# ZHKKKe/PixelSSL

Measured on NVIDIA H100. Metric: images/sec DeepLab-v2-R101 MT 513x513 bs16, higher is better.
Workload: dtype f16x3 (fp16 pairs, fp32 accumulate)

## Files before the change

pixelssl_b200/csrc/conv_tc.cu:

```cuda
#include "common.cuh"
#include <cuda.h>
#include <cstdlib>

typedef CUresult (*EncodeTiledFn)(CUtensorMap*, CUtensorMapDataType, cuuint32_t, void*, const cuuint64_t*,
                                  const cuuint64_t*, const cuuint32_t*, const cuuint32_t*, CUtensorMapInterleave,
                                  CUtensorMapSwizzle, CUtensorMapL2promotion, CUtensorMapFloatOOBfill);
static EncodeTiledFn get_encode() {
    static EncodeTiledFn fn = nullptr;
    if (!fn) {
        void* p = nullptr;
        cudaDriverEntryPointQueryResult q;
        if (cudaGetDriverEntryPoint("cuTensorMapEncodeTiled", &p, cudaEnableDefault, &q) == cudaSuccess &&
            q == cudaDriverEntryPointSuccess)
            fn = (EncodeTiledFn)p;
    }
    return fn;
}

static int make_act_map(CUtensorMap* m, const void* base, int C, int W, int H, int N, int bw, int bh, int estride = 1, int f16 = 0) {
    EncodeTiledFn enc = get_encode();
    if (!enc) return PXL_ERR_UNSUPPORTED;
    const cuuint64_t eb = f16 ? 2 : 4;
    cuuint64_t dims[4] = {(cuuint64_t)C, (cuuint64_t)W, (cuuint64_t)H, (cuuint64_t)N};
    cuuint64_t strides[3] = {(cuuint64_t)C * eb, (cuuint64_t)W * C * eb, (cuuint64_t)H * W * C * eb};
// ... 6 lines not shown
    return r == CUDA_SUCCESS ? 0 : PXL_ERR_BAD_ARG;
}

static int make_w_map(CUtensorMap* m, const void* base, int64_t K, int rows, int bn, int f16 = 0) {
    EncodeTiledFn enc = get_encode();
    if (!enc) return PXL_ERR_UNSUPPORTED;
    cuuint64_t dims[2] = {(cuuint64_t)K, (cuuint64_t)rows};
    cuuint64_t strides[1] = {(cuuint64_t)K * (f16 ? 2 : 4)};
    cuuint32_t box[2] = {(cuuint32_t)(f16 ? 64 : 32), (cuuint32_t)bn};
    cuuint32_t es[2] = {1, 1};
    CUresult r = enc(m, f16 ? CU_TENSOR_MAP_DATA_TYPE_FLOAT16 : CU_TENSOR_MAP_DATA_TYPE_FLOAT32, 2, (void*)base, dims, strides, box, es,
                     CU_TENSOR_MAP_INTERLEAVE_NONE, CU_TENSOR_MAP_SWIZZLE_128B, CU_TENSOR_MAP_L2_PROMOTION_L2_256B,
                     CU_TENSOR_MAP_FLOAT_OOB_FILL_NONE);
    return r == CUDA_SUCCESS ? 0 : PXL_ERR_BAD_ARG;
}

__device__ __forceinline__ uint32_t smem_u32(const void* p) { return (uint32_t)__cvta_generic_to_shared(p); }

__device__ __forceinline__ void mbar_init(uint64_t* bar, uint32_t count) {
    asm volatile("mbarrier.init.shared::cta.b64 [%0], %1;" ::"r"(smem_u32(bar)), "r"(count));
}
__device__ __forceinline__ void mbar_expect_tx(uint64_t* bar, uint32_t bytes) {
    asm volatile("mbarrier.arrive.expect_tx.shared::cta.b64 _, [%0], %1;" ::"r"(smem_u32(bar)), "r"(bytes) : "memory");
}
__device__ __forceinline__ void mbar_arrive(uint64_t* bar) {
    asm volatile("mbarrier.arrive.shared::cta.b64 _, [%0];" ::"r"(smem_u32(bar)) : "memory");
}
__device__ __forceinline__ bool mbar_try_wait(uint64_t* bar, uint32_t parity) {
    uint32_t ok;
    asm volatile(
        "{\n\t.reg .pred p;\n\t"
        "mbarrier.try_wait.parity.shared::cta.b64 p, [%1], %2;\n\t"
        "selp.u32 %0, 1, 0, p;\n\t}"
        : "=r"(ok)
        : "r"(smem_u32(bar)), "r"(parity)
        : "memory");
    return ok != 0;
}
__device__ __forceinline__ bool mbar_wait(uint64_t* bar, uint32_t parity, int* flag, int code) {
    for (uint32_t spin = 0; spin < (1u << 22); ++spin) {
        if (mbar_try_wait(bar, parity)) return true;
        if ((spin & 1023u) == 1023u && *(volatile int*)flag != 0) return false;
    }
    atomicCAS(flag, 0, code);
    return false;
}
__device__ __forceinline__ void tma_load_4d(void* dst, const CUtensorMap* map, uint64_t* bar, int c0, int c1, int c2, int c3) {
    asm volatile(
        "cp.async.bulk.tensor.4d.shared::cluster.global.mbarrier::complete_tx::bytes [%0], [%1, {%3, %4, %5, %6}], [%2];"
        ::"r"(smem_u32(dst)), "l"(map), "r"(smem_u32(bar)), "r"(c0), "r"(c1), "r"(c2), "r"(c3)
        : "memory");
}
__device__ __forceinline__ void tma_load_2d(void* dst, const CUtensorMap* map, uint64_t* bar, int c0, int c1) {
    asm volatile(
        "cp.async.bulk.tensor.2d.shared::cluster.global.mbarrier::complete_tx::bytes [%0], [%1, {%3, %4}], [%2];"
        ::"r"(smem_u32(dst)), "l"(map), "r"(smem_u32(bar)), "r"(c0), "r"(c1)
        : "memory");
}
__device__ __forceinline__ bool elect_one() {
    uint32_t pred = 0;
    asm volatile(
        "{\n\t.reg .b32 rx;\n\t.reg .pred px;\n\t"
        "elect.sync rx|px, 0xffffffff;\n\t"
        "@px mov.s32 %0, 1;\n\t}"
        : "+r"(pred));
    return pred != 0;
}
__device__ __forceinline__ void named_bar(int id, int count) {
    asm volatile("bar.sync %0, %1;" ::"r"(id), "r"(count) : "memory");
}
__device__ __forceinline__ void fence_async_smem() { asm volatile("fence.proxy.async.shared::cta;" ::: "memory"); }

__device__ __forceinline__ uint64_t sw128_desc(uint32_t smem_addr, uint32_t lbo_bytes = 16) {
    uint64_t d = 0;
    d |= (uint64_t)((smem_addr & 0x3FFFF) >> 4);
    d |= (uint64_t)((lbo_bytes >> 4) & 0x3FFF) << 16;
    d |= (uint64_t)(1024 >> 4) << 32;
    d |= (uint64_t)1 << 62;
    return d;
}
__device__ __forceinline__ void wg_arrive() { asm volatile("wgmma.fence.sync.aligned;" ::: "memory"); }
__device__ __forceinline__ void wg_commit() { asm volatile("wgmma.commit_group.sync.aligned;" ::: "memory"); }
__device__ __forceinline__ void wg_wait0() { asm volatile("wgmma.wait_group.sync.aligned 0;" ::: "memory"); }
template <int R>
__device__ __forceinline__ void fence_regs(float (&d)[R]) {
#pragma unroll
    for (int i = 0; i < R; ++i) asm volatile("" : "+f"(d[i])::"memory");
}

template <int N, int KIND>
__device__ __forceinline__ void wgmma_op(float (&d)[N / 2], uint64_t da, uint64_t db, int scale_d);
template <> __device__ __forceinline__ void wgmma_op<32, 0>(float (&d)[16], uint64_t da, uint64_t db, int scale_d) {
    asm volatile(
        "{\n\t.reg .pred p;\n\tsetp.ne.b32 p, %18, 0;\n\t"
        "wgmma.mma_async.sync.aligned.m64n32k8.f32.tf32.tf32 {%0, %1, %2, %3, %4, %5, %6, %7, %8, %9, %10, %11, %12, %13, %14, %15}, %16, %17, p, 1, 1;\n\t}"
        : "+f"(d[0]), "+f"(d[1]), "+f"(d[2]), "+f"(d[3]), "+f"(d[4]), "+f"(d[5]), "+f"(d[6]), "+f"(d[7]), "+f"(d[8]), "+f"(d[9]), "+f"(d[10]), "+f"(d[11]), "+f"(d[12]), "+f"(d[13]), "+f"(d[14]), "+f"(d[15])
        : "l"(da), "l"(db), "r"(scale_d));
}
template <> __device__ __forceinline__ void wgmma_op<64, 0>(float (&d)[32], uint64_t da, uint64_t db, int scale_d) {
    asm volatile(
        "{\n\t.reg .pred p;\n\tsetp.ne.b32 p, %34, 0;\n\t"
        "wgmma.mma_async.sync.aligned.m64n64k8.f32.tf32.tf32 {%0, %1, %2, %3, %4, %5, %6, %7, %8, %9, %10, %11, %12, %13, %14, %15, %16, %17, %18, %19, %20, %21, %22, %23, %24, %25, %26, %27, %28, %29, %30, %31}, %32, %33, p, 1, 1;\n\t}"
        : "+f"(d[0]), "+f"(d[1]), "+f"(d[2]), "+f"(d[3]), "+f"(d[4]), "+f"(d[5]), "+f"(d[6]), "+f"(d[7]), "+f"(d[8]), "+f"(d[9]), "+f"(d[10]), "+f"(d[11]), "+f"(d[12]), "+f"(d[13]), "+f"(d[14]), "+f"(d[15]), "+f"(d[16]), "+f"(d[17]), "+f"(d[18]), "+f"(d[19]), "+f"(d[20]), "+f"(d[21]), "+f"(d[22]), "+f"(d[23]), "+f"(d[24]), "+f"(d[25]), "+f"(d[26]), "+f"(d[27]), "+f"(d[28]), "+f"(d[29]), "+f"(d[30]), "+f"(d[31])
        : "l"(da), "l"(db), "r"(scale_d));
}
template <> __device__ __forceinline__ void wgmma_op<128, 0>(float (&d)[64], uint64_t da, uint64_t db, int scale_d) {
    asm volatile(
        "{\n\t.reg .pred p;\n\tsetp.ne.b32 p, %66, 0;\n\t"
        "wgmma.mma_async.sync.aligned.m64n128k8.f32.tf32.tf32 {%0, %1, %2, %3, %4, %5, %6, %7, %8, %9, %10, %11, %12, %13, %14, %15, %16, %17, %18, %19, %20, %21, %22, %23, %24, %25, %26, %27, %28, %29, %30, %31, %32, %33, %34, %35, %36, %37, %38, %39, %40, %41, %42, %43, %44, %45, %46, %47, %48, %49, %50, %51, %52, %53, %54, %55, %56, %57, %58, %59, %60, %61, %62, %63}, %64, %65, p, 1, 1;\n\t}"
        : "+f"(d[0]), "+f"(d[1]), "+f"(d[2]), "+f"(d[3]), "+f"(d[4]), "+f"(d[5]), "+f"(d[6]), "+f"(d[7]), "+f"(d[8]), "+f"(d[9]), "+f"(d[10]), "+f"(d[11]), "+f"(d[12]), "+f"(d[13]), "+f"(d[14]), "+f"(d[15]), "+f"(d[16]), "+f"(d[17]), "+f"(d[18]), "+f"(d[19]), "+f"(d[20]), "+f"(d[21]), "+f"(d[22]), "+f"(d[23]), "+f"(d[24]), "+f"(d[25]), "+f"(d[26]), "+f"(d[27]), "+f"(d[28]), "+f"(d[29]), "+f"(d[30]), "+f"(d[31]), "+f"(d[32]), "+f"(d[33]), "+f"(d[34]), "+f"(d[35]), "+f"(d[36]), "+f"(d[37]), "+f"(d[38]), "+f"(d[39]), "+f"(d[40]), "+f"(d[41]), "+f"(d[42]), "+f"(d[43]), "+f"(d[44]), "+f"(d[45]), "+f"(d[46]), "+f"(d[47]), "+f"(d[48]), "+f"(d[49]), "+f"(d[50]), "+f"(d[51]), "+f"(d[52]), "+f"(d[53]), "+f"(d[54]), "+f"(d[55]), "+f"(d[56]), "+f"(d[57]), "+f"(d[58]), "+f"(d[59]), "+f"(d[60]), "+f"(d[61]), "+f"(d[62]), "+f"(d[63])
        : "l"(da), "l"(db), "r"(scale_d));
}
template <> __device__ __forceinline__ void wgmma_op<32, 1>(float (&d)[16], uint64_t da, uint64_t db, int scale_d) {
    asm volatile(
        "{\n\t.reg .pred p;\n\tsetp.ne.b32 p, %18, 0;\n\t"
        "wgmma.mma_async.sync.aligned.m64n32k16.f32.f16.f16 {%0, %1, %2, %3, %4, %5, %6, %7, %8, %9, %10, %11, %12, %13, %14, %15}, %16, %17, p, 1, 1, 0, 0;\n\t}"
        : "+f"(d[0]), "+f"(d[1]), "+f"(d[2]), "+f"(d[3]), "+f"(d[4]), "+f"(d[5]), "+f"(d[6]), "+f"(d[7]), "+f"(d[8]), "+f"(d[9]), "+f"(d[10]), "+f"(d[11]), "+f"(d[12]), "+f"(d[13]), "+f"(d[14]), "+f"(d[15])
        : "l"(da), "l"(db), "r"(scale_d));
}
template <> __device__ __forceinline__ void wgmma_op<64, 1>(float (&d)[32], uint64_t da, uint64_t db, int scale_d) {
    asm volatile(
        "{\n\t.reg .pred p;\n\tsetp.ne.b32 p, %34, 0;\n\t"
        "wgmma.mma_async.sync.aligned.m64n64k16.f32.f16.f16 {%0, %1, %2, %3, %4, %5, %6, %7, %8, %9, %10, %11, %12, %13, %14, %15, %16, %17, %18, %19, %20, %21, %22, %23, %24, %25, %26, %27, %28, %29, %30, %31}, %32, %33, p, 1, 1, 0, 0;\n\t}"
        : "+f"(d[0]), "+f"(d[1]), "+f"(d[2]), "+f"(d[3]), "+f"(d[4]), "+f"(d[5]), "+f"(d[6]), "+f"(d[7]), "+f"(d[8]), "+f"(d[9]), "+f"(d[10]), "+f"(d[11]), "+f"(d[12]), "+f"(d[13]), "+f"(d[14]), "+f"(d[15]), "+f"(d[16]), "+f"(d[17]), "+f"(d[18]), "+f"(d[19]), "+f"(d[20]), "+f"(d[21]), "+f"(d[22]), "+f"(d[23]), "+f"(d[24]), "+f"(d[25]), "+f"(d[26]), "+f"(d[27]), "+f"(d[28]), "+f"(d[29]), "+f"(d[30]), "+f"(d[31])
        : "l"(da), "l"(db), "r"(scale_d));
}
template <> __device__ __forceinline__ void wgmma_op<128, 1>(float (&d)[64], uint64_t da, uint64_t db, int scale_d) {
    asm volatile(
        "{\n\t.reg .pred p;\n\tsetp.ne.b32 p, %66, 0;\n\t"
        "wgmma.mma_async.sync.aligned.m64n128k16.f32.f16.f16 {%0, %1, %2, %3, %4, %5, %6, %7, %8, %9, %10, %11, %12, %13, %14, %15, %16, %17, %18, %19, %20, %21, %22, %23, %24, %25, %26, %27, %28, %29, %30, %31, %32, %33, %34, %35, %36, %37, %38, %39, %40, %41, %42, %43, %44, %45, %46, %47, %48, %49, %50, %51, %52, %53, %54, %55, %56, %57, %58, %59, %60, %61, %62, %63}, %64, %65, p, 1, 1, 0, 0;\n\t}"
        : "+f"(d[0]), "+f"(d[1]), "+f"(d[2]), "+f"(d[3]), "+f"(d[4]), "+f"(d[5]), "+f"(d[6]), "+f"(d[7]), "+f"(d[8]), "+f"(d[9]), "+f"(d[10]), "+f"(d[11]), "+f"(d[12]), "+f"(d[13]), "+f"(d[14]), "+f"(d[15]), "+f"(d[16]), "+f"(d[17]), "+f"(d[18]), "+f"(d[19]), "+f"(d[20]), "+f"(d[21]), "+f"(d[22]), "+f"(d[23]), "+f"(d[24]), "+f"(d[25]), "+f"(d[26]), "+f"(d[27]), "+f"(d[28]), "+f"(d[29]), "+f"(d[30]), "+f"(d[31]), "+f"(d[32]), "+f"(d[33]), "+f"(d[34]), "+f"(d[35]), "+f"(d[36]), "+f"(d[37]), "+f"(d[38]), "+f"(d[39]), "+f"(d[40]), "+f"(d[41]), "+f"(d[42]), "+f"(d[43]), "+f"(d[44]), "+f"(d[45]), "+f"(d[46]), "+f"(d[47]), "+f"(d[48]), "+f"(d[49]), "+f"(d[50]), "+f"(d[51]), "+f"(d[52]), "+f"(d[53]), "+f"(d[54]), "+f"(d[55]), "+f"(d[56]), "+f"(d[57]), "+f"(d[58]), "+f"(d[59]), "+f"(d[60]), "+f"(d[61]), "+f"(d[62]), "+f"(d[63])
        : "l"(da), "l"(db), "r"(scale_d));
}
template <> __device__ __forceinline__ void wgmma_op<64, 2>(float (&d)[32], uint64_t da, uint64_t db, int scale_d) {
    asm volatile(
        "{\n\t.reg .pred p;\n\tsetp.ne.b32 p, %34, 0;\n\t"
        "wgmma.mma_async.sync.aligned.m64n64k16.f32.f16.f16 {%0, %1, %2, %3, %4, %5, %6, %7, %8, %9, %10, %11, %12, %13, %14, %15, %16, %17, %18, %19, %20, %21, %22, %23, %24, %25, %26, %27, %28, %29, %30, %31}, %32, %33, p, 1, 1, 1, 1;\n\t}"
        : "+f"(d[0]), "+f"(d[1]), "+f"(d[2]), "+f"(d[3]), "+f"(d[4]), "+f"(d[5]), "+f"(d[6]), "+f"(d[7]), "+f"(d[8]), "+f"(d[9]), "+f"(d[10]), "+f"(d[11]), "+f"(d[12]), "+f"(d[13]), "+f"(d[14]), "+f"(d[15]), "+f"(d[16]), "+f"(d[17]), "+f"(d[18]), "+f"(d[19]), "+f"(d[20]), "+f"(d[21]), "+f"(d[22]), "+f"(d[23]), "+f"(d[24]), "+f"(d[25]), "+f"(d[26]), "+f"(d[27]), "+f"(d[28]), "+f"(d[29]), "+f"(d[30]), "+f"(d[31])
        : "l"(da), "l"(db), "r"(scale_d));
}
template <> __device__ __forceinline__ void wgmma_op<128, 2>(float (&d)[64], uint64_t da, uint64_t db, int scale_d) {
    asm volatile(
        "{\n\t.reg .pred p;\n\tsetp.ne.b32 p, %66, 0;\n\t"
        "wgmma.mma_async.sync.aligned.m64n128k16.f32.f16.f16 {%0, %1, %2, %3, %4, %5, %6, %7, %8, %9, %10, %11, %12, %13, %14, %15, %16, %17, %18, %19, %20, %21, %22, %23, %24, %25, %26, %27, %28, %29, %30, %31, %32, %33, %34, %35, %36, %37, %38, %39, %40, %41, %42, %43, %44, %45, %46, %47, %48, %49, %50, %51, %52, %53, %54, %55, %56, %57, %58, %59, %60, %61, %62, %63}, %64, %65, p, 1, 1, 1, 1;\n\t}"
        : "+f"(d[0]), "+f"(d[1]), "+f"(d[2]), "+f"(d[3]), "+f"(d[4]), "+f"(d[5]), "+f"(d[6]), "+f"(d[7]), "+f"(d[8]), "+f"(d[9]), "+f"(d[10]), "+f"(d[11]), "+f"(d[12]), "+f"(d[13]), "+f"(d[14]), "+f"(d[15]), "+f"(d[16]), "+f"(d[17]), "+f"(d[18]), "+f"(d[19]), "+f"(d[20]), "+f"(d[21]), "+f"(d[22]), "+f"(d[23]), "+f"(d[24]), "+f"(d[25]), "+f"(d[26]), "+f"(d[27]), "+f"(d[28]), "+f"(d[29]), "+f"(d[30]), "+f"(d[31]), "+f"(d[32]), "+f"(d[33]), "+f"(d[34]), "+f"(d[35]), "+f"(d[36]), "+f"(d[37]), "+f"(d[38]), "+f"(d[39]), "+f"(d[40]), "+f"(d[41]), "+f"(d[42]), "+f"(d[43]), "+f"(d[44]), "+f"(d[45]), "+f"(d[46]), "+f"(d[47]), "+f"(d[48]), "+f"(d[49]), "+f"(d[50]), "+f"(d[51]), "+f"(d[52]), "+f"(d[53]), "+f"(d[54]), "+f"(d[55]), "+f"(d[56]), "+f"(d[57]), "+f"(d[58]), "+f"(d[59]), "+f"(d[60]), "+f"(d[61]), "+f"(d[62]), "+f"(d[63])
        : "l"(da), "l"(db), "r"(scale_d));
}

template <int BN, int F16>
__device__ __forceinline__ void mma_slice(float (&part)[BN / 2], float (&corr)[BN / 2], uint64_t da, uint64_t db, uint64_t dal,
                                          uint64_t dbl, bool split3) {
#pragma unroll
    for (int k = 0; k < 4; ++k) wgmma_op<BN, F16>(part, da + 2 * k, db + 2 * k, k);
    if (split3) {
#pragma unroll
        for (int k = 0; k < 4; ++k) wgmma_op<BN, F16>(corr, dal + 2 * k, db + 2 * k, k);
#pragma unroll
        for (int k = 0; k < 4; ++k) wgmma_op<BN, F16>(corr, da + 2 * k, dbl + 2 * k, 1);
    }
}

__device__ __forceinline__ float4 tf32_split4(float4 v, float4& lo) {
    float4 h;
    const float* vp = &v.x; float* hp = &h.x; float* lp = &lo.x;
#pragma unroll
    for (int e = 0; e < 4; ++e) {
        uint32_t u;
        asm("cvt.rna.tf32.f32 %0, %1;" : "=r"(u) : "f"(vp[e]));
        u &= 0xFFFFE000u;
        hp[e] = __uint_as_float(u);
        lp[e] = vp[e] - hp[e];
    }
    return h;
}

struct TcParams {
    int Cin, Cout, ldo, ntaps, kchunks;
    int N, OH, OW;
    int BW, BH, tilesW, tilesH;
    int stages, nsplit;
    int a_inkernel;
    int in_mul;
    int out_mul, out_offy, out_offx, outH, outW;
    int ntilesN, pix_tiles, total_tiles;
    int kc;
    float out_scale;
    int out_acc;
    short dy[PXL_MAX_TAPS], dx[PXL_MAX_TAPS], widx[PXL_MAX_TAPS];
};

#define TC_A_BYTES (128 * 128)
#define TC_MAX_STAGES 8
#define TC_THREADS 384

__device__ __forceinline__ void tc_tile_coords(const TcParams& p, int tile, int bn, int& n0, int& w0, int& h0, int& n) {
    const int nt = tile / p.pix_tiles, pix = tile - nt * p.pix_tiles;
    const int tw = pix % p.tilesW, th = (pix / p.tilesW) % p.tilesH;
    n = pix / (p.tilesW * p.tilesH);
    w0 = tw * p.BW; h0 = th * p.BH; n0 = nt * bn;
}

template <int BN, int F16>
__global__ void __launch_bounds__(TC_THREADS, 1)
conv_wg_kernel(const __grid_constant__ CUtensorMap mapA, const __grid_constant__ CUtensorMap mapAlo,
               const __grid_constant__ CUtensorMap mapB, const __grid_constant__ CUtensorMap mapBlo,
               const TcParams p, const float* __restrict__ bias, float* __restrict__ out,
               double* __restrict__ stats, int* __restrict__ err_flag, const float* __restrict__ oscale_ptr) {
    extern __shared__ __align__(1024) uint8_t smem_raw[];
    __shared__ uint64_t full_bar[TC_MAX_STAGES], empty_bar[TC_MAX_STAGES];
    __shared__ float st_warp[2][8][BN];

    uint8_t* smem = (uint8_t*)(((uintptr_t)smem_raw + 1023) & ~(uintptr_t)1023);
    constexpr int B_BYTES = BN * 128;
    constexpr int PER_OP = TC_A_BYTES + B_BYTES;
    const int stage_bytes = PER_OP * (p.nsplit == 3 ? 2 : 1);
    const int iters = p.ntaps * p.kchunks;

    if (threadIdx.x == 0) {
        for (int s = 0; s < p.stages; ++s) { mbar_init(&full_bar[s], 1); mbar_init(&empty_bar[s], 256); }
        asm volatile("fence.mbarrier_init.release.cluster;" ::: "memory");
    }
    __syncthreads();
    PXL_PDL_SYNC();

    if (threadIdx.x < 128) {
        asm volatile("setmaxnreg.dec.sync.aligned.u32 40;" ::: "memory");
        if (threadIdx.x >= 32) return;
        uint32_t tx = (uint32_t)((p.BW * p.BH * 128 + B_BYTES) * (p.nsplit == 3 ? 2 : 1));
        if (p.a_inkernel) tx -= (uint32_t)(p.BW * p.BH * 128);
        uint32_t s = 0, ph = 0;
        bool ok = true;
        for (int tile = blockIdx.x; tile < p.total_tiles && ok; tile += gridDim.x) {
            int n0, w0, h0, n;
            tc_tile_coords(p, tile, BN, n0, w0, h0, n);
            int tap = 0, c0 = 0;
            for (int it = 0; it < iters; ++it) {
                ok = __all_sync(0xffffffffu, mbar_wait(&empty_bar[s], ph ^ 1u, err_flag, 1));
                if (!ok) break;
                uint8_t* sa = smem + (size_t)s * stage_bytes;
                const int ax = w0 * p.in_mul + p.dx[tap], ay = h0 * p.in_mul + p.dy[tap];
                const int bk = p.widx[tap] * p.Cin + c0;
                if (elect_one()) {
                    mbar_expect_tx(&full_bar[s], tx);
                    tma_load_4d(sa, &mapA, &full_bar[s], c0, ax, ay, n);
                    tma_load_2d(sa + TC_A_BYTES, &mapB, &full_bar[s], bk, n0);
                    if (p.nsplit == 3) {
                        if (!p.a_inkernel) tma_load_4d(sa + PER_OP, &mapAlo, &full_bar[s], c0, ax, ay, n);
                        tma_load_2d(sa + PER_OP + TC_A_BYTES, &mapBlo, &full_bar[s], bk, n0);
                    }
                }
                __syncwarp();
                c0 += p.kc; if (c0 >= p.Cin) { c0 = 0; ++tap; }
                if (++s == (uint32_t)p.stages) { s = 0; ph ^= 1u; }
            }
        }
        return;
    }

    asm volatile("setmaxnreg.inc.sync.aligned.u32 232;" ::: "memory");
    const int ct = threadIdx.x - 128;
    const int cw = ct >> 7, t = ct & 127;
    const int warp = t >> 5, lane = t & 31;
    const float osc = p.out_scale * (oscale_ptr ? __ldg(oscale_ptr) : 1.f);
    const uint32_t smem_base = smem_u32(smem);
    const bool split3 = p.nsplit == 3;
    float acc[BN / 2], part[BN / 2], corr[BN / 2];
    uint32_t s = 0, ph = 0;
    int st_n0 = -1;
    float st_s = 0.f, st_q = 0.f;
    bool ok = true;
    auto flush_stats = [&]() {
        if (st_n0 >= 0 && ct < BN && st_n0 + ct < p.Cout && (st_s != 0.f || st_q != 0.f)) {
            atomicAdd(stats + st_n0 + ct, (double)st_s);
            atomicAdd(stats + p.Cout + st_n0 + ct, (double)st_q);
        }
        st_s = 0.f; st_q = 0.f;
    };
    for (int tile = blockIdx.x; tile < p.total_tiles && ok; tile += gridDim.x) {
        int n0, w0, h0, n;
        tc_tile_coords(p, tile, BN, n0, w0, h0, n);
        if (stats && n0 != st_n0) { flush_stats(); st_n0 = n0; }
#pragma unroll
        for (int i = 0; i < BN / 2; ++i) acc[i] = 0.f;
        for (int it = 0; it < iters; ++it) {
            ok = __all_sync(0xffffffffu, mbar_wait(&full_bar[s], ph, err_flag, 2));
            if (!ok) break;
            uint8_t* sa = smem + (size_t)s * stage_bytes;
            if (p.a_inkernel) {
                float4* a_hi = reinterpret_cast<float4*>(sa + cw * (TC_A_BYTES / 2));
                float4* a_lo = reinterpret_cast<float4*>(sa + PER_OP + cw * (TC_A_BYTES / 2));
#pragma unroll
                for (int c = 0; c < TC_A_BYTES / 2 / 16 / 128; ++c) {
                    float4 lo;
                    const float4 hi = tf32_split4(a_hi[t + c * 128], lo);
                    a_hi[t + c * 128] = hi;
                    a_lo[t + c * 128] = lo;
                }
                fence_async_smem();
                named_bar(2 + cw, 128);
            }
            const uint32_t sa32 = smem_base + s * (uint32_t)stage_bytes;
            const uint32_t arow = (uint32_t)cw * (TC_A_BYTES / 2);
            const uint64_t da = sw128_desc(sa32 + arow), db = sw128_desc(sa32 + TC_A_BYTES);
            const uint64_t dal = sw128_desc(sa32 + PER_OP + arow), dbl = sw128_desc(sa32 + PER_OP + TC_A_BYTES);
            wg_arrive();
            fence_regs(part);
            fence_regs(corr);
#pragma unroll
            for (int k = 0; k < 2; ++k) wgmma_op<BN, F16>(part, da + 2 * k, db + 2 * k, k);
            if (split3) {
#pragma unroll
                for (int k = 0; k < 4; ++k) wgmma_op<BN, F16>(corr, dal + 2 * k, db + 2 * k, k);
#pragma unroll
                for (int k = 0; k < 4; ++k) wgmma_op<BN, F16>(corr, da + 2 * k, dbl + 2 * k, 1);
            }
            wg_commit();
            wg_wait0();
            fence_regs(part);
#pragma unroll
            for (int i = 0; i < BN / 2; ++i) acc[i] += part[i];
            wg_arrive();
            fence_regs(part);
#pragma unroll
            for (int k = 2; k < 4; ++k) wgmma_op<BN, F16>(part, da + 2 * k, db + 2 * k, k - 2);
            wg_commit();
            wg_wait0();
            fence_regs(part);
            fence_regs(corr);
            mbar_arrive(&empty_bar[s]);
            if (split3) {
#pragma unroll
                for (int i = 0; i < BN / 2; ++i) acc[i] += part[i] + corr[i];
            } else {
#pragma unroll
                for (int i = 0; i < BN / 2; ++i) acc[i] += part[i];
            }
            if (++s == (uint32_t)p.stages) { s = 0; ph ^= 1u; }
        }
        if (!ok) break;
        int64_t obase[2];
        bool valid[2];
#pragma unroll
        for (int h = 0; h < 2; ++h) {
            const int r = cw * 64 + warp * 16 + (lane >> 2) + 8 * h;
            const int hy = r / p.BW, wx = r - hy * p.BW;
            const int oy = h0 + hy, ox = w0 + wx;
            valid[h] = hy < p.BH && oy < p.OH && ox < p.OW;
            obase[h] = ((int64_t)(n * p.outH + oy * p.out_mul + p.out_offy) * p.outW + ox * p.out_mul + p.out_offx) * p.ldo;
        }
        const bool vec2 = (p.ldo & 1) == 0 && ((uintptr_t)out & 7) == 0;
#pragma unroll
        for (int j = 0; j < BN / 8; ++j) {
            const int cl = j * 8 + 2 * (lane & 3);
            const int col = n0 + cl;
            const bool c0ok = col < p.Cout, c1ok = col + 1 < p.Cout;
            const float b0 = (bias && c0ok) ? __ldg(bias + col) : 0.f, b1 = (bias && c1ok) ? __ldg(bias + col + 1) : 0.f;
            float v[2][2];
#pragma unroll
            for (int h = 0; h < 2; ++h) {
                v[h][0] = acc[j * 4 + 2 * h] * osc + b0;
                v[h][1] = acc[j * 4 + 2 * h + 1] * osc + b1;
                if (!valid[h]) continue;
                float* o = out + obase[h] + col;
                if (p.out_acc) {
                    if (c0ok) o[0] += v[h][0];
                    if (c1ok) o[1] += v[h][1];
                } else if (c1ok && vec2) {
                    *reinterpret_cast<float2*>(o) = make_float2(v[h][0], v[h][1]);
                } else {
                    if (c0ok) o[0] = v[h][0];
                    if (c1ok) o[1] = v[h][1];
                }
            }
            if (stats) {
                float s0 = (valid[0] ? v[0][0] : 0.f) + (valid[1] ? v[1][0] : 0.f);
                float s1 = (valid[0] ? v[0][1] : 0.f) + (valid[1] ? v[1][1] : 0.f);
                float q0 = (valid[0] ? v[0][0] * v[0][0] : 0.f) + (valid[1] ? v[1][0] * v[1][0] : 0.f);
                float q1 = (valid[0] ? v[0][1] * v[0][1] : 0.f) + (valid[1] ? v[1][1] * v[1][1] : 0.f);
#pragma unroll
                for (int o = 4; o < 32; o <<= 1) {
                    s0 += __shfl_xor_sync(0xffffffffu, s0, o); s1 += __shfl_xor_sync(0xffffffffu, s1, o);
                    q0 += __shfl_xor_sync(0xffffffffu, q0, o); q1 += __shfl_xor_sync(0xffffffffu, q1, o);
                }
                if (lane < 4) {
                    const int slot = cw * 4 + warp;
                    st_warp[0][slot][cl] = s0; st_warp[0][slot][cl + 1] = s1;
                    st_warp[1][slot][cl] = q0; st_warp[1][slot][cl + 1] = q1;
                }
            }
        }
        if (stats) {
            named_bar(1, 256);
            if (ct < BN) {
#pragma unroll
                for (int w8 = 0; w8 < 8; ++w8) { st_s += st_warp[0][w8][ct]; st_q += st_warp[1][w8][ct]; }
            }
            named_bar(1, 256);
        }
    }
    if (stats && ok) flush_stats();
}

__global__ void __launch_bounds__(256)
split_tf32_kernel(const float4* __restrict__ x, float4* __restrict__ hi, float4* __restrict__ lo, int64_t n4) {
    const int64_t stride = (int64_t)gridDim.x * blockDim.x;
    for (int64_t i = (int64_t)blockIdx.x * blockDim.x + threadIdx.x; i < n4; i += stride) {
        float4 l;
        hi[i] = tf32_split4(__ldcs(x + i), l);
        lo[i] = l;
    }
}

extern "C" int pxl_split_tf32(const float* x, float* hi, float* lo, int64_t n, void* stream) {
    if (!x || !hi || !lo || n <= 0 || (n & 3)) return PXL_ERR_BAD_ARG;
    const int64_t n4 = n / 4;
    int blocks = (int)(pxl_cdiv(n4, 256 * 2) < PXL_NUM_SMS * 8 ? pxl_cdiv(n4, 256 * 2) : PXL_NUM_SMS * 8);
    split_tf32_kernel<<<blocks, 256, 0, (cudaStream_t)stream>>>((const float4*)x, (float4*)hi, (float4*)lo, n4);
    PXL_CHECK_LAUNCH();
    return 0;
}

static int* g_err_flag = nullptr;

static int ensure_err_flag() {
    if (g_err_flag) return 0;
    cudaError_t e = cudaMalloc(&g_err_flag, sizeof(int));
    if (e != cudaSuccess) return (int)e;
    e = cudaMemset(g_err_flag, 0, sizeof(int));
    return e == cudaSuccess ? 0 : (int)e;
}

template <typename K>
static int query_dyn_smem_limit(K kernel) {
    int dev = 0, optin = 0;
    cudaFuncAttributes a;
    if (cudaGetDevice(&dev) != cudaSuccess || cudaDeviceGetAttribute(&optin, cudaDevAttrMaxSharedMemoryPerBlockOptin, dev) != cudaSuccess ||
        cudaFuncGetAttributes(&a, kernel) != cudaSuccess)
        return 0;
    return optin - (int)a.sharedSizeBytes;
}

static void pick_tile(int OH, int OW, bool flat, int& BW, int& BH) {
    if (flat) { BW = 128; BH = 1; return; }
    double best = -1.0;
    BW = 16; BH = 8;
    for (int bw = 4; bw <= 128 && bw <= 256; ++bw) {
        int bh = 128 / bw;
        if (bh < 1) break;
        if (bh > 256) bh = 256;
        const int64_t tiles = (int64_t)((OW + bw - 1) / bw) * ((OH + bh - 1) / bh);
        const double eff = (double)OH * OW / ((double)tiles * 128.0);
        if (eff > best + 1e-9) { best = eff; BW = bw; BH = bh; }
    }
}

template <int BN, int F16>
static int fwd_smem_limit() {
    static const int v = query_dyn_smem_limit(conv_wg_kernel<BN, F16>);
    return v;
}

template <int BN, int F16>
static int launch_fwd(const CUtensorMap& mA, const CUtensorMap& mAlo, const CUtensorMap& mB, const CUtensorMap& mBlo,
                      const TcParams& p, size_t smem, cudaStream_t st, const float* bias, float* out, double* stats,
                      const float* oscale_ptr) {
    static bool attr = false;
    if (!attr) {
        cudaError_t e = cudaFuncSetAttribute(conv_wg_kernel<BN, F16>, cudaFuncAttributeMaxDynamicSharedMemorySize, fwd_smem_limit<BN, F16>());
        if (e != cudaSuccess) return (int)e;
        attr = true;
// ... 64 lines not shown
        const int64_t M = (int64_t)g->N * g->H * g->W;
        if (M >= (1ll << 31)) return PXL_ERR_UNSUPPORTED;
        p.N = 1; p.OH = 1; p.OW = (int)M;
        mapW = (int)M; mapH = 1; mapN = 1;
        p.outH = 1; p.outW = (int)M;
    } else {
        p.N = g->N; p.OH = g->OH; p.OW = g->OW;
        mapW = g->W; mapH = g->H; mapN = g->N;
        p.outH = has_out_xform ? ext->out_H : g->OH; p.outW = has_out_xform ? ext->out_W : g->OW;
    }
    pick_tile(p.OH, p.OW, flat, p.BW, p.BH);
    if (g->mul == 2 && (p.BW > 128 || p.BH > 128)) return PXL_ERR_UNSUPPORTED;
    const int BN = g->Cout > 64 ? 128 : (g->Cout > 32 ? 64 : 32);
    const int stage_bytes = (TC_A_BYTES + BN * 128) * (nsplit == 3 ? 2 : 1);
    p.tilesW = (p.OW + p.BW - 1) / p.BW; p.tilesH = (p.OH + p.BH - 1) / p.BH;
    p.pix_tiles = p.N * p.tilesH * p.tilesW;
    p.ntilesN = (g->Cout + BN - 1) / BN;
    const int64_t n_tiles = (int64_t)p.pix_tiles * p.ntilesN;
    if (n_tiles >= (1ll << 31)) return PXL_ERR_UNSUPPORTED;
    p.total_tiles = (int)n_tiles;
    const int smem_limit = f16 ? (BN == 128 ? fwd_smem_limit<128, 1>() : BN == 64 ? fwd_smem_limit<64, 1>() : fwd_smem_limit<32, 1>())
                               : (BN == 128 ? fwd_smem_limit<128, 0>() : BN == 64 ? fwd_smem_limit<64, 0>() : fwd_smem_limit<32, 0>());
    if (smem_limit <= 0) return PXL_ERR_UNSUPPORTED;
    p.stages = (smem_limit - 1024) / stage_bytes;
    if (p.stages > TC_MAX_STAGES) p.stages = TC_MAX_STAGES;
    if (p.stages < 2) return PXL_ERR_UNSUPPORTED;
    const size_t smem = (size_t)p.stages * stage_bytes + 1024;

    CUtensorMap mA, mAlo, mB, mBlo;
    int rc = make_act_map(&mA, in_hi, g->Cin, mapW, mapH, mapN, p.BW, p.BH, g->mul, f16);
    if (rc) return rc;
    rc = make_w_map(&mB, w_hi, (int64_t)wtaps * g->Cin, g->Cout, BN, f16);
    if (rc) return rc;
    if (nsplit == 3) {
        if (a_inkernel) mAlo = mA;
        else {
            rc = make_act_map(&mAlo, in_lo, g->Cin, mapW, mapH, mapN, p.BW, p.BH, g->mul, f16);
            if (rc) return rc;
        }
        rc = make_w_map(&mBlo, w_lo, (int64_t)wtaps * g->Cin, g->Cout, BN, f16);
        if (rc) return rc;
    } else {
        mAlo = mA; mBlo = mB;
    }
    p.out_acc = (ext && ext->out_accumulate) ? 1 : 0;
    if ((rc = ensure_err_flag())) return rc;
    cudaStream_t st = (cudaStream_t)stream;
    double* st_ptr = ext ? (double*)ext->bn_stats : nullptr;
    if (f16) {
        if (BN == 128) return launch_fwd<128, 1>(mA, mAlo, mB, mBlo, p, smem, st, bias, out, st_ptr, oscale_ptr);
        if (BN == 64) return launch_fwd<64, 1>(mA, mAlo, mB, mBlo, p, smem, st, bias, out, st_ptr, oscale_ptr);
        return launch_fwd<32, 1>(mA, mAlo, mB, mBlo, p, smem, st, bias, out, st_ptr, oscale_ptr);
    }
    if (BN == 128) return launch_fwd<128, 0>(mA, mAlo, mB, mBlo, p, smem, st, bias, out, st_ptr, oscale_ptr);
    if (BN == 64) return launch_fwd<64, 0>(mA, mAlo, mB, mBlo, p, smem, st, bias, out, st_ptr, oscale_ptr);
    return launch_fwd<32, 0>(mA, mAlo, mB, mBlo, p, smem, st, bias, out, st_ptr, oscale_ptr);
}

extern "C" int pxl_conv_tc_status(void) {
    if (!g_err_flag) return 0;
    int v = 0;
    if (cudaMemcpy(&v, g_err_flag, sizeof(int), cudaMemcpyDeviceToHost) != cudaSuccess) return -1;
    return v;
}

extern "C" int pxl_conv_tc_impl(const pxl_conv_geom* g, const int* taps, const float* in, const float* w,
                                const float* bias, float* out, void* stream) {
    if (!g) return PXL_ERR_BAD_ARG;
    if (g->precision == 2) return PXL_ERR_UNSUPPORTED;
    return pxl_conv_tc_launch(g, taps, in, nullptr, w, nullptr, bias, out, stream);
}

struct WgParams {
    int Cin, Cout, ldo, ntaps;
    int N, OH, OW, mul;
    int BW, BH, tilesW, tilesH, rows, rows_alloc;
    int stages, nsplit;
    int inkernel;
    int slab_ch;
    float out_scale;
    int tiles_ci, ktiles_per_cta, ktiles_total;
    short dy[PXL_MAX_TAPS], dx[PXL_MAX_TAPS];
};

template <int BN, int F16>
__global__ void __launch_bounds__(TC_THREADS, 1)
conv_wgrad_wg_kernel(const __grid_constant__ CUtensorMap mapDy, const __grid_constant__ CUtensorMap mapDyLo,
                     const __grid_constant__ CUtensorMap mapX, const __grid_constant__ CUtensorMap mapXLo,
                     const WgParams p, float* __restrict__ dw, float* __restrict__ ws, int* __restrict__ err_flag,
                     const float* __restrict__ oscale_ptr) {
    extern __shared__ __align__(1024) uint8_t smem_raw[];
    __shared__ uint64_t full_bar[TC_MAX_STAGES], empty_bar[TC_MAX_STAGES];
    uint8_t* smem = (uint8_t*)(((uintptr_t)smem_raw + 1023) & ~(uintptr_t)1023);

    const int slab_bytes = p.rows_alloc * 128;
    const int slabsA = 128 / p.slab_ch;
    const int slabsB = BN / p.slab_ch;
    const int per_op = (slabsA + slabsB) * slab_bytes;
    const int stage_bytes = per_op * (p.nsplit == 3 ? 2 : 1);
    constexpr int KT_BYTES = (128 + BN) * 128;
    uint8_t* kt = smem + (size_t)p.stages * stage_bytes;
    const int tile_co = blockIdx.x / p.tiles_ci, tile_ci = blockIdx.x % p.tiles_ci;
    const int co0 = tile_co * 128, ci0 = tile_ci * BN;
    const int tap = blockIdx.y;
    const int kt0 = blockIdx.z * p.ktiles_per_cta;
    int kt1 = kt0 + p.ktiles_per_cta;
    if (kt1 > p.ktiles_total) kt1 = p.ktiles_total;
    const int iters = kt1 - kt0;
    int nsA = (p.ldo - co0 + p.slab_ch - 1) / p.slab_ch; if (nsA > slabsA) nsA = slabsA;
    int nsB = (p.Cin - ci0 + p.slab_ch - 1) / p.slab_ch; if (nsB > slabsB) nsB = slabsB;

    {
        uint4 z = make_uint4(0, 0, 0, 0);
        const int total16 = p.stages * stage_bytes / 16;
        for (int i = threadIdx.x; i < total16; i += blockDim.x) reinterpret_cast<uint4*>(smem)[i] = z;
        fence_async_smem();
    }
    if (threadIdx.x == 0) {
        for (int s = 0; s < p.stages; ++s) { mbar_init(&full_bar[s], 1); mbar_init(&empty_bar[s], 256); }
        asm volatile("fence.mbarrier_init.release.cluster;" ::: "memory");
    }
    __syncthreads();
    PXL_PDL_SYNC();
    if (iters <= 0) return;

    if (threadIdx.x < 128) {
        asm volatile("setmaxnreg.dec.sync.aligned.u32 40;" ::: "memory");
        if (threadIdx.x >= 32) return;
        const uint32_t box_bytes = (uint32_t)(p.rows * 128);
        const int nparts = (p.nsplit == 3 && !p.inkernel) ? 2 : 1;
        const uint32_t tx = box_bytes * (uint32_t)(nsA + nsB) * (uint32_t)nparts;
        const int tdy = p.dy[tap], tdx = p.dx[tap];
        int tw = kt0 % p.tilesW, th = (kt0 / p.tilesW) % p.tilesH, n = kt0 / (p.tilesW * p.tilesH);
        uint32_t s = 0, ph = 0;
        for (int it = 0; it < iters; ++it) {
            if (!__all_sync(0xffffffffu, mbar_wait(&empty_bar[s], ph ^ 1u, err_flag, 11))) break;
            const int w0 = tw * p.BW, h0 = th * p.BH;
            uint8_t* sa = smem + (size_t)s * stage_bytes;
            if (elect_one()) {
                mbar_expect_tx(&full_bar[s], tx);
                for (int part = 0; part < nparts; ++part) {
                    uint8_t* base = sa + (size_t)part * per_op;
                    const CUtensorMap* mdy = part ? &mapDyLo : &mapDy;
                    const CUtensorMap* mx = part ? &mapXLo : &mapX;
                    for (int j = 0; j < nsA; ++j)
                        tma_load_4d(base + (size_t)j * slab_bytes, mdy, &full_bar[s], co0 + p.slab_ch * j, w0, h0, n);
                    for (int j = 0; j < nsB; ++j)
                        tma_load_4d(base + (size_t)(slabsA + j) * slab_bytes, mx, &full_bar[s], ci0 + p.slab_ch * j,
                                    w0 * p.mul + tdx, h0 * p.mul + tdy, n);
                }
            }
            __syncwarp();
            if (++tw == p.tilesW) { tw = 0; if (++th == p.tilesH) { th = 0; ++n; } }
            if (++s == (uint32_t)p.stages) { s = 0; ph ^= 1u; }
        }
        return;
    }

    asm volatile("setmaxnreg.inc.sync.aligned.u32 232;" ::: "memory");
    const int ct = threadIdx.x - 128;
    const int cw = ct >> 7, t = ct & 127;
    const int warp = t >> 5, lane = t & 31;
    const bool split3 = p.nsplit == 3;
    const uint32_t smem_base = smem_u32(smem);
    float acc[BN / 2], part[BN / 2], corr[BN / 2];
#pragma unroll
    for (int i = 0; i < BN / 2; ++i) acc[i] = 0.f;
    uint32_t s = 0, ph = 0;
    bool ok = true;
    for (int it = 0; it < iters; ++it) {
        ok = __all_sync(0xffffffffu, mbar_wait(&full_bar[s], ph, err_flag, 12));
        if (!ok) break;
        uint8_t* sa = smem + (size_t)s * stage_bytes;
        const uint32_t sa32 = smem_base + s * (uint32_t)stage_bytes;
        if constexpr (F16 != 0) {
            const int kmma = p.rows_alloc / 16;
            const uint32_t sb32 = sa32 + (uint32_t)(slabsA * slab_bytes);
            const uint64_t da = sw128_desc(sa32 + (uint32_t)(cw * slab_bytes), (uint32_t)slab_bytes);
            const uint64_t db = sw128_desc(sb32, (uint32_t)slab_bytes);
            const uint64_t dal = sw128_desc(sa32 + (uint32_t)per_op + (uint32_t)(cw * slab_bytes), (uint32_t)slab_bytes);
            const uint64_t dbl = sw128_desc(sb32 + (uint32_t)per_op, (uint32_t)slab_bytes);
            const uint64_t kstep = (16 * 128) >> 4;
            wg_arrive();
            fence_regs(part);
            fence_regs(corr);
            for (int k = 0; k < kmma; ++k) wgmma_op<BN, 2>(part, da + kstep * k, db + kstep * k, k);
            if (split3) {
                for (int k = 0; k < kmma; ++k) wgmma_op<BN, 2>(corr, dal + kstep * k, db + kstep * k, k);
                for (int k = 0; k < kmma; ++k) wgmma_op<BN, 2>(corr, da + kstep * k, dbl + kstep * k, 1);
            }
            wg_commit();
            wg_wait0();
            fence_regs(part);
            fence_regs(corr);
            mbar_arrive(&empty_bar[s]);
        } else {
            named_bar(1, 256);
            const int units = (128 + BN) * 8;
            for (int u = ct; u < units; u += 256) {
                const int R = u >> 3, g = u & 7;
                const int slab = R < 128 ? (R >> 5) : slabsA + ((R - 128) >> 5);
                const int c = R & 31;
                const uint8_t* src = sa + (size_t)slab * slab_bytes + (c & 3) * 4;
                float4 v, vl = make_float4(0.f, 0.f, 0.f, 0.f);
                float* vp = &v.x; float* lp = &vl.x;
#pragma unroll
                for (int e = 0; e < 4; ++e) {
                    const int px = 4 * g + e;
                    const int off = px * 128 + ((((c >> 2) ^ (px & 7))) << 4);
                    vp[e] = *reinterpret_cast<const float*>(src + off);
                    if (split3 && !p.inkernel) lp[e] = *reinterpret_cast<const float*>(src + per_op + off);
                }
                if (p.inkernel) v = tf32_split4(v, vl);
                const int doff = R * 128 + ((g ^ (R & 7)) << 4);
                *reinterpret_cast<float4*>(kt + doff) = v;
                if (split3) *reinterpret_cast<float4*>(kt + KT_BYTES + doff) = vl;
            }
            fence_async_smem();
            named_bar(1, 256);
            mbar_arrive(&empty_bar[s]);
            const uint32_t k32 = smem_u32(kt);
            const uint32_t arow = (uint32_t)cw * 64 * 128;
            const uint64_t da = sw128_desc(k32 + arow), db = sw128_desc(k32 + 128 * 128);
            const uint64_t dal = sw128_desc(k32 + KT_BYTES + arow), dbl = sw128_desc(k32 + KT_BYTES + 128 * 128);
            wg_arrive();
            fence_regs(part);
            fence_regs(corr);
            mma_slice<BN, 0>(part, corr, da, db, dal, dbl, split3);
            wg_commit();
            wg_wait0();
            fence_regs(part);
            fence_regs(corr);
        }
        if (split3) {
#pragma unroll
            for (int i = 0; i < BN / 2; ++i) acc[i] += part[i] + corr[i];
        } else {
#pragma unroll
            for (int i = 0; i < BN / 2; ++i) acc[i] += part[i];
        }
        if (++s == (uint32_t)p.stages) { s = 0; ph ^= 1u; }
    }
    if (!ok) return;
    const float osc = p.out_scale * (oscale_ptr ? __ldg(oscale_ptr) : 1.f);
#pragma unroll
    for (int h = 0; h < 2; ++h) {
        const int co = co0 + cw * 64 + warp * 16 + (lane >> 2) + 8 * h;
        if (co >= p.Cout) continue;
        const int64_t row = ((int64_t)co * p.ntaps + tap) * p.Cin;
        float* drow = gridDim.z == 1 ? dw + row : ws + (int64_t)blockIdx.z * p.Cout * p.ntaps * p.Cin + row;
#pragma unroll
        for (int j = 0; j < BN / 8; ++j) {
            const int ci = ci0 + j * 8 + 2 * (lane & 3);
            const float v0 = acc[j * 4 + 2 * h] * osc, v1 = acc[j * 4 + 2 * h + 1] * osc;
            if (gridDim.z == 1) {
                if (ci < p.Cin) drow[ci] += v0;
                if (ci + 1 < p.Cin) drow[ci + 1] += v1;
            } else {
                if (ci < p.Cin) drow[ci] = v0;
                if (ci + 1 < p.Cin) drow[ci + 1] = v1;
            }
        }
    }
}

__global__ void __launch_bounds__(256)
wgrad_reduce_kernel(const float* __restrict__ ws, float* __restrict__ dw, int64_t n, int splits) {
    const int64_t stride = (int64_t)gridDim.x * blockDim.x;
    for (int64_t i = (int64_t)blockIdx.x * blockDim.x + threadIdx.x; i < n; i += stride) {
        float s = __ldg(ws + i);
        for (int z = 1; z < splits; ++z) s += __ldg(ws + (int64_t)z * n + i);
        dw[i] += s;
    }
}

// ... 160 lines not shown
```

Measured before the change: 159.6.

## Overlap WGMMA groups in f16 conv mainloop, unroll wgrad MMAs, shuffle-reduce BN stats

In the fp16 forward conv mainloop, WGMMA commit groups are split and retired with wait_group 1, so accumulation of one partial overlaps the next group's MMAs. In the non-split path the smem stage release is deferred across iterations. The BN-statistics epilogue replaces the per-value xor-shuffle reduction with a reduce-scatter over pairs of columns, cutting shuffle count. The wgrad f16 path dispatches on the MMA count to fully unrolled templates instead of a runtime loop. The cost is more code and more complex stage-release ordering, which raises the risk of hazards.

```diff
diff --git a/pixelssl_b200/csrc/conv_tc.cu b/pixelssl_b200/csrc/conv_tc.cu
--- a/pixelssl_b200/csrc/conv_tc.cu
+++ b/pixelssl_b200/csrc/conv_tc.cu
@@ -112,6 +112,7 @@
 __device__ __forceinline__ void wg_arrive() { asm volatile("wgmma.fence.sync.aligned;" ::: "memory"); }
 __device__ __forceinline__ void wg_commit() { asm volatile("wgmma.commit_group.sync.aligned;" ::: "memory"); }
 __device__ __forceinline__ void wg_wait0() { asm volatile("wgmma.wait_group.sync.aligned 0;" ::: "memory"); }
+__device__ __forceinline__ void wg_wait1() { asm volatile("wgmma.wait_group.sync.aligned 1;" ::: "memory"); }
 template <int R>
 __device__ __forceinline__ void fence_regs(float (&d)[R]) {
 #pragma unroll
@@ -202,6 +203,16 @@
         lp[e] = vp[e] - hp[e];
     }
     return h;
+}
+
+template <int H, int R>
+__device__ __forceinline__ void reduce_scatter_step(float (&v)[R], int lane, int o) {
+    const bool up = (lane & o) != 0;
+#pragma unroll
+    for (int i = 0; i < H; ++i) {
+        const float keep = up ? v[H + i] : v[i], send = up ? v[i] : v[H + i];
+        v[i] = keep + __shfl_xor_sync(0xffffffffu, send, o);
+    }
 }
 
 struct TcParams {
@@ -312,60 +323,133 @@
         if (stats && n0 != st_n0) { flush_stats(); st_n0 = n0; }
 #pragma unroll
         for (int i = 0; i < BN / 2; ++i) acc[i] = 0.f;
-        for (int it = 0; it < iters; ++it) {
-            ok = __all_sync(0xffffffffu, mbar_wait(&full_bar[s], ph, err_flag, 2));
-            if (!ok) break;
-            uint8_t* sa = smem + (size_t)s * stage_bytes;
-            if (p.a_inkernel) {
-                float4* a_hi = reinterpret_cast<float4*>(sa + cw * (TC_A_BYTES / 2));
-                float4* a_lo = reinterpret_cast<float4*>(sa + PER_OP + cw * (TC_A_BYTES / 2));
-#pragma unroll
-                for (int c = 0; c < TC_A_BYTES / 2 / 16 / 128; ++c) {
-                    float4 lo;
-                    const float4 hi = tf32_split4(a_hi[t + c * 128], lo);
-                    a_hi[t + c * 128] = hi;
-                    a_lo[t + c * 128] = lo;
+        if constexpr (F16 != 0) {
+            int rel = -1;
+            for (int it = 0; it < iters; ++it) {
+                ok = __all_sync(0xffffffffu, mbar_wait(&full_bar[s], ph, err_flag, 2));
+                if (!ok) break;
+                const uint32_t sa32 = smem_base + s * (uint32_t)stage_bytes;
+                const uint32_t arow = (uint32_t)cw * (TC_A_BYTES / 2);
+                const uint64_t da = sw128_desc(sa32 + arow), db = sw128_desc(sa32 + TC_A_BYTES);
+                const bool last = it == iters - 1;
+                if (split3) {
+                    const uint64_t dal = sw128_desc(sa32 + PER_OP + arow), dbl = sw128_desc(sa32 + PER_OP + TC_A_BYTES);
+                    fence_regs(part);
+                    fence_regs(corr);
+                    wg_arrive();
+                    wgmma_op<BN, 1>(part, da, db, 0);
+                    wgmma_op<BN, 1>(part, da + 2, db + 2, 1);
+                    wg_commit();
+#pragma unroll
+                    for (int k = 0; k < 4; ++k) wgmma_op<BN, 1>(corr, dal + 2 * k, db + 2 * k, k);
+#pragma unroll
+                    for (int k = 0; k < 4; ++k) wgmma_op<BN, 1>(corr, da + 2 * k, dbl + 2 * k, 1);
+                    wg_commit();
+                    wg_wait1();
+                    fence_regs(part);
+#pragma unroll
+                    for (int i = 0; i < BN / 2; ++i) acc[i] += part[i];
+                    fence_regs(part);
+                    wg_arrive();
+                    wgmma_op<BN, 1>(part, da + 4, db + 4, 0);
+                    wgmma_op<BN, 1>(part, da + 6, db + 6, 1);
+                    wg_commit();
+                    wg_wait0();
+                    mbar_arrive(&empty_bar[s]);
+                    fence_regs(part);
+                    fence_regs(corr);
+#pragma unroll
+                    for (int i = 0; i < BN / 2; ++i) acc[i] += part[i] + corr[i];
+                } else {
+                    fence_regs(part);
+                    wg_arrive();
+                    wgmma_op<BN, 1>(part, da, db, 0);
+                    wgmma_op<BN, 1>(part, da + 2, db + 2, 1);
+                    wg_commit();
+                    if (rel >= 0) {
+                        wg_wait1();
+                        mbar_arrive(&empty_bar[rel]);
+                        fence_regs(corr);
+#pragma unroll
+                        for (int i = 0; i < BN / 2; ++i) acc[i] += corr[i];
+                    }
+                    fence_regs(corr);
+                    wg_arrive();
+                    wgmma_op<BN, 1>(corr, da + 4, db + 4, 0);
+                    wgmma_op<BN, 1>(corr, da + 6, db + 6, 1);
+                    wg_commit();
+                    wg_wait1();
+                    fence_regs(part);
+#pragma unroll
+                    for (int i = 0; i < BN / 2; ++i) acc[i] += part[i];
+                    rel = (int)s;
+                    if (last) {
+                        wg_wait0();
+                        mbar_arrive(&empty_bar[s]);
+                        rel = -1;
+                        fence_regs(corr);
+#pragma unroll
+                        for (int i = 0; i < BN / 2; ++i) acc[i] += corr[i];
+                    }
                 }
-                fence_async_smem();
-                named_bar(2 + cw, 128);
+                if (++s == (uint32_t)p.stages) { s = 0; ph ^= 1u; }
             }
-            const uint32_t sa32 = smem_base + s * (uint32_t)stage_bytes;
-            const uint32_t arow = (uint32_t)cw * (TC_A_BYTES / 2);
-            const uint64_t da = sw128_desc(sa32 + arow), db = sw128_desc(sa32 + TC_A_BYTES);
-            const uint64_t dal = sw128_desc(sa32 + PER_OP + arow), dbl = sw128_desc(sa32 + PER_OP + TC_A_BYTES);
-            wg_arrive();
-            fence_regs(part);
-            fence_regs(corr);
-#pragma unroll
-            for (int k = 0; k < 2; ++k) wgmma_op<BN, F16>(part, da + 2 * k, db + 2 * k, k);
-            if (split3) {
-#pragma unroll
-                for (int k = 0; k < 4; ++k) wgmma_op<BN, F16>(corr, dal + 2 * k, db + 2 * k, k);
-#pragma unroll
-                for (int k = 0; k < 4; ++k) wgmma_op<BN, F16>(corr, da + 2 * k, dbl + 2 * k, 1);
+        } else {
+            for (int it = 0; it < iters; ++it) {
+                ok = __all_sync(0xffffffffu, mbar_wait(&full_bar[s], ph, err_flag, 2));
+                if (!ok) break;
+                uint8_t* sa = smem + (size_t)s * stage_bytes;
+                if (p.a_inkernel) {
+                    float4* a_hi = reinterpret_cast<float4*>(sa + cw * (TC_A_BYTES / 2));
+                    float4* a_lo = reinterpret_cast<float4*>(sa + PER_OP + cw * (TC_A_BYTES / 2));
+#pragma unroll
+                    for (int c = 0; c < TC_A_BYTES / 2 / 16 / 128; ++c) {
+                        float4 lo;
+                        const float4 hi = tf32_split4(a_hi[t + c * 128], lo);
+                        a_hi[t + c * 128] = hi;
+                        a_lo[t + c * 128] = lo;
+                    }
+                    fence_async_smem();
+                    named_bar(2 + cw, 128);
+                }
+                const uint32_t sa32 = smem_base + s * (uint32_t)stage_bytes;
+                const uint32_t arow = (uint32_t)cw * (TC_A_BYTES / 2);
+                const uint64_t da = sw128_desc(sa32 + arow), db = sw128_desc(sa32 + TC_A_BYTES);
+                const uint64_t dal = sw128_desc(sa32 + PER_OP + arow), dbl = sw128_desc(sa32 + PER_OP + TC_A_BYTES);
+                wg_arrive();
+                fence_regs(part);
+                fence_regs(corr);
+#pragma unroll
+                for (int k = 0; k < 2; ++k) wgmma_op<BN, F16>(part, da + 2 * k, db + 2 * k, k);
+                if (split3) {
+#pragma unroll
+                    for (int k = 0; k < 4; ++k) wgmma_op<BN, F16>(corr, dal + 2 * k, db + 2 * k, k);
+#pragma unroll
+                    for (int k = 0; k < 4; ++k) wgmma_op<BN, F16>(corr, da + 2 * k, dbl + 2 * k, 1);
+                }
+                wg_commit();
+                wg_wait0();
+                fence_regs(part);
+#pragma unroll
+                for (int i = 0; i < BN / 2; ++i) acc[i] += part[i];
+                wg_arrive();
+                fence_regs(part);
+#pragma unroll
+                for (int k = 2; k < 4; ++k) wgmma_op<BN, F16>(part, da + 2 * k, db + 2 * k, k - 2);
+                wg_commit();
+                wg_wait0();
+                fence_regs(part);
+                fence_regs(corr);
+                mbar_arrive(&empty_bar[s]);
+                if (split3) {
+#pragma unroll
+                    for (int i = 0; i < BN / 2; ++i) acc[i] += part[i] + corr[i];
+                } else {
+#pragma unroll
+                    for (int i = 0; i < BN / 2; ++i) acc[i] += part[i];
+                }
+                if (++s == (uint32_t)p.stages) { s = 0; ph ^= 1u; }
             }
-            wg_commit();
-            wg_wait0();
-            fence_regs(part);
-#pragma unroll
-            for (int i = 0; i < BN / 2; ++i) acc[i] += part[i];
-            wg_arrive();
-            fence_regs(part);
-#pragma unroll
-            for (int k = 2; k < 4; ++k) wgmma_op<BN, F16>(part, da + 2 * k, db + 2 * k, k - 2);
-            wg_commit();
-            wg_wait0();
-            fence_regs(part);
-            fence_regs(corr);
-            mbar_arrive(&empty_bar[s]);
-            if (split3) {
-#pragma unroll
-                for (int i = 0; i < BN / 2; ++i) acc[i] += part[i] + corr[i];
-            } else {
-#pragma unroll
-                for (int i = 0; i < BN / 2; ++i) acc[i] += part[i];
-            }
-            if (++s == (uint32_t)p.stages) { s = 0; ph ^= 1u; }
         }
         if (!ok) break;
         int64_t obase[2];
@@ -379,6 +463,7 @@
             obase[h] = ((int64_t)(n * p.outH + oy * p.out_mul + p.out_offy) * p.outW + ox * p.out_mul + p.out_offx) * p.ldo;
         }
         const bool vec2 = (p.ldo & 1) == 0 && ((uintptr_t)out & 7) == 0;
+        float red[8];
 #pragma unroll
         for (int j = 0; j < BN / 8; ++j) {
             const int cl = j * 8 + 2 * (lane & 3);
@@ -407,15 +492,14 @@
                 float s1 = (valid[0] ? v[0][1] : 0.f) + (valid[1] ? v[1][1] : 0.f);
                 float q0 = (valid[0] ? v[0][0] * v[0][0] : 0.f) + (valid[1] ? v[1][0] * v[1][0] : 0.f);
                 float q1 = (valid[0] ? v[0][1] * v[0][1] : 0.f) + (valid[1] ? v[1][1] * v[1][1] : 0.f);
-#pragma unroll
-                for (int o = 4; o < 32; o <<= 1) {
-                    s0 += __shfl_xor_sync(0xffffffffu, s0, o); s1 += __shfl_xor_sync(0xffffffffu, s1, o);
-                    q0 += __shfl_xor_sync(0xffffffffu, q0, o); q1 += __shfl_xor_sync(0xffffffffu, q1, o);
-                }
-                if (lane < 4) {
-                    const int slot = cw * 4 + warp;
-                    st_warp[0][slot][cl] = s0; st_warp[0][slot][cl + 1] = s1;
-                    st_warp[1][slot][cl] = q0; st_warp[1][slot][cl + 1] = q1;
+                const int r = (j & 1) * 4;
+                red[r + 0] = s0; red[r + 1] = s1; red[r + 2] = q0; red[r + 3] = q1;
+                if (j & 1) {
+                    reduce_scatter_step<4>(red, lane, 4);
+                    reduce_scatter_step<2>(red, lane, 8);
+                    reduce_scatter_step<1>(red, lane, 16);
+                    const int idx = ((lane >> 2) & 1) * 4 + ((lane >> 3) & 1) * 2 + ((lane >> 4) & 1), kind = idx & 3;
+                    st_warp[kind >> 1][cw * 4 + warp][(j - 1 + (idx >> 2)) * 8 + 2 * (lane & 3) + (kind & 1)] = red[0];
                 }
             }
         }
@@ -646,6 +730,23 @@
     int tiles_ci, ktiles_per_cta, ktiles_total;
     short dy[PXL_MAX_TAPS], dx[PXL_MAX_TAPS];
 };
+
+template <int BN, int KM, bool SPLIT3>
+__device__ __forceinline__ void wgrad_h16_mmas(float (&part)[BN / 2], float (&corr)[BN / 2], uint64_t da, uint64_t db,
+                                               uint64_t dal, uint64_t dbl) {
+    constexpr uint64_t kstep = (16 * 128) >> 4;
+    wg_arrive();
+#pragma unroll
+    for (int k = 0; k < KM; ++k) wgmma_op<BN, 2>(part, da + kstep * k, db + kstep * k, k);
+    if (SPLIT3) {
+#pragma unroll
+        for (int k = 0; k < KM; ++k) wgmma_op<BN, 2>(corr, dal + kstep * k, db + kstep * k, k);
+#pragma unroll
+        for (int k = 0; k < KM; ++k) wgmma_op<BN, 2>(corr, da + kstep * k, dbl + kstep * k, 1);
+    }
+    wg_commit();
+    wg_wait0();
+}
 
 template <int BN, int F16>
 __global__ void __launch_bounds__(TC_THREADS, 1)
@@ -744,17 +845,27 @@
             const uint64_t db = sw128_desc(sb32, (uint32_t)slab_bytes);
             const uint64_t dal = sw128_desc(sa32 + (uint32_t)per_op + (uint32_t)(cw * slab_bytes), (uint32_t)slab_bytes);
             const uint64_t dbl = sw128_desc(sb32 + (uint32_t)per_op, (uint32_t)slab_bytes);
-            const uint64_t kstep = (16 * 128) >> 4;
-            wg_arrive();
             fence_regs(part);
             fence_regs(corr);
-            for (int k = 0; k < kmma; ++k) wgmma_op<BN, 2>(part, da + kstep * k, db + kstep * k, k);
             if (split3) {
-                for (int k = 0; k < kmma; ++k) wgmma_op<BN, 2>(corr, dal + kstep * k, db + kstep * k, k);
-                for (int k = 0; k < kmma; ++k) wgmma_op<BN, 2>(corr, da + kstep * k, dbl + kstep * k, 1);
+                switch (kmma) {
+                    case 1: wgrad_h16_mmas<BN, 1, true>(part, corr, da, db, dal, dbl); break;
+                    case 2: wgrad_h16_mmas<BN, 2, true>(part, corr, da, db, dal, dbl); break;
+                    case 3: wgrad_h16_mmas<BN, 3, true>(part, corr, da, db, dal, dbl); break;
+                    default: wgrad_h16_mmas<BN, 4, true>(part, corr, da, db, dal, dbl); break;
+                }
+            } else {
+                switch (kmma) {
+                    case 1: wgrad_h16_mmas<BN, 1, false>(part, corr, da, db, dal, dbl); break;
+                    case 2: wgrad_h16_mmas<BN, 2, false>(part, corr, da, db, dal, dbl); break;
+                    case 3: wgrad_h16_mmas<BN, 3, false>(part, corr, da, db, dal, dbl); break;
+                    case 4: wgrad_h16_mmas<BN, 4, false>(part, corr, da, db, dal, dbl); break;
+                    case 5: wgrad_h16_mmas<BN, 5, false>(part, corr, da, db, dal, dbl); break;
+                    case 6: wgrad_h16_mmas<BN, 6, false>(part, corr, da, db, dal, dbl); break;
+                    case 7: wgrad_h16_mmas<BN, 7, false>(part, corr, da, db, dal, dbl); break;
+                    default: wgrad_h16_mmas<BN, 8, false>(part, corr, da, db, dal, dbl); break;
+                }
             }
-            wg_commit();
-            wg_wait0();
             fence_regs(part);
             fence_regs(corr);
             mbar_arrive(&empty_bar[s]);
```

After: 166.2 (median of 6 runs). +4.2%, better.
